# angeladai/sgnn

Measured on AMD Instinct MI355X. Metric: TSDF blocks/sec fwd+bwd (64^3@5% occ, bs32), higher is better.
Workload: dtype f32

## Files before the change

### sgnn_amd/csrc/conv.hip

```cpp
#include <stdlib.h>
#include "common.h"

#include "conv_common.h"

#define CONV_SMALL_GRID ((int64_t)((g_tune.conv_small_rows + CONV_ROWS_PER_BLOCK - 1) / CONV_ROWS_PER_BLOCK))

template <int CIN, int COUT, int M, bool EX, bool WEPI>
__device__ __forceinline__ void conv_fwd_body(const float *__restrict__ x, int64_t n_in,
                                              const float *__restrict__ w, const int32_t *__restrict__ table,
                                              int64_t ld, int K, int64_t n_out, float *y, int flags,
                                              int in_shift, const ConvEx &ex, const ConvEpi &epi, int wg_cap) {
  using C = ConvCfg<CIN, COUT>;
  constexpr int V = C::V, CINP = C::CINP, NT = C::NT, KC = C::KC;
  constexpr int RPW = 16 * M;
  __shared__ __attribute__((aligned(16))) float wl[KC * C::PER_K];
  __shared__ double sred[4 * 2 * NT * 16];
  static_assert(!WEPI || (NT == 1 && M == 4 && !EX && COUT % 4 == 0), "wide epilogue: one column tile of whole 16-byte chunks");
  __shared__ float ecst[WEPI ? 64 : 1];

  const int tid = threadIdx.x, lane = tid & 63, wave = tid >> 6;
  const int r = lane & 15, q = lane >> 4;
  const unsigned groups = EX ? (unsigned)ex.groups : 1u;
  unsigned nwg = gridDim.x;
  if (epi.n_dev) n_out = sgnn_dyn_n(n_out, epi.n_dev);
// ... 144 lines not shown
      load_b(0, b0);
      int kk = 0;
      for (; kk + 1 < kc; kk += 2) {
        gather(iv1, a1);
        const int32_t iv3 = idx_at(k0 + kk + 3);
        load_b(kk + 1, b1);
        __builtin_amdgcn_sched_barrier(0);
        mma_b(a0, b0);
        __builtin_amdgcn_sched_barrier(0);
        gather(iv2, a0);
        iv1 = iv3;
        iv2 = idx_at(k0 + kk + 4);
        load_b(kk + 2 < kc ? kk + 2 : kc - 1, b0);
        __builtin_amdgcn_sched_barrier(0);
        mma_b(a1, b1);
        __builtin_amdgcn_sched_barrier(0);
      }
      if constexpr (WEPI) {
        __builtin_amdgcn_sched_barrier(0);
        if constexpr (SGNN_WEPI_EARLY != 0) conv_epi_wide_prefetch<COUT, M>(erows, row0, n_out, epi, epi.stats, x, SGNN_WEPI_EARLY);
        __builtin_amdgcn_sched_barrier(0);
      }
      if (kk < kc) mma_b(a0, b0);
    }
  }

  if constexpr (WEPI)
    conv_epi_wide_finish<COUT, M>(acc, erows, row0, n_out, y, epi, epi.stats, ecst, s1, s2, x);
  else
    conv_epilogue_rows<COUT, M, NT>(acc, row0, n_out, groups, grp, y, epi, EX ? 0 : epi.stats, x, s1, s2);
  }
  conv_epilogue_stats<COUT, NT>(s1, s2, epi, EX ? 0 : epi.stats, sred, blockIdx.x);
}

template <int CIN, int COUT, int M, bool EX>
__global__ __launch_bounds__(256) void k_conv_fwd(const float *__restrict__ x, int64_t n_in,
                                                 const float *__restrict__ w, const int32_t *__restrict__ table,
                                                 int64_t ld, int K, int64_t n_out, float *y, int flags,
                                                 int in_shift, ConvEx ex, ConvEpi epi, int wg_cap) {
  conv_fwd_body<CIN, COUT, M, EX, false>(x, n_in, w, table, ld, K, n_out, y, flags, in_shift, ex, epi, wg_cap);
}

template <int CIN, int COUT>
__global__ __launch_bounds__(256) __attribute__((amdgpu_waves_per_eu(4, 8))) void k_conv_fwd_w(
    const float *__restrict__ x, int64_t n_in, const float *__restrict__ w, const int32_t *__restrict__ table, int64_t ld,
    int K, int64_t n_out, float *y, int flags, int in_shift, ConvEx ex, ConvEpi epi, int wg_cap) {
  conv_fwd_body<CIN, COUT, CONV_MREP, false, true>(x, n_in, w, table, ld, K, n_out, y, flags, in_shift, ex, epi, wg_cap);
}

template <int CIN, int COUT>
__global__ __launch_bounds__(256) void k_conv_small(const float *__restrict__ x, int64_t n_in,
                                                   const float *__restrict__ w, const int32_t *__restrict__ table,
                                                   int64_t ld, int K, int64_t n_out, float *y, int flags, int in_shift,
                                                   ConvEpi epi) {
  using C = ConvCfg<CIN, COUT>;
  constexpr int V = C::V, CINP = C::CINP, NT = C::NT;
  constexpr int KW = 7;
  __shared__ float red[4][NT * 256];
  __shared__ double sred[4][2][NT * 16];
  const int tid = threadIdx.x, lane = tid & 63, wave = tid >> 6;
  const int r = lane & 15, q = lane >> 4;
  const int64_t row0 = (int64_t)blockIdx.x * 16;
  if (epi.n_dev) {
    n_out = sgnn_dyn_n(n_out, epi.n_dev);
    if (row0 >= n_out) {
      if (epi.stats)
        for (int o = tid; o < 2 * COUT; o += 256) epi.partial[(size_t)blockIdx.x * 2 * COUT + o] = 0.0;
      return;
    }
  }
  const bool transpose = flags & SGNN_CONV_TRANSPOSE_W, flip = flags & SGNN_CONV_FLIP_K;
  const int per = (K + 3) >> 2;
  const int k0 = wave * per;
  const int nk = (K - k0) < per ? ((K - k0) > 0 ? (K - k0) : 0) : per;

  const uint32_t ldx4 = (uint32_t)epi.ldx * 4u, ldy4 = (uint32_t)epi.ldy * 4u;
  const __amdgpu_buffer_rsrc_t rs_x = make_rsrc(x, (uint32_t)(((n_in - 1) * epi.ldx + CIN) * 4));
  const __amdgpu_buffer_rsrc_t rs_t = make_rsrc(table, (uint32_t)((int64_t)K * ld * 4));
  const __amdgpu_buffer_rsrc_t rs_y = make_rsrc(y, (uint32_t)(((n_out - 1) * epi.ldy + COUT) * 4));
  const uint32_t lane_off = (uint32_t)(row0 + r) * 4u;
  const uint32_t ld4 = (uint32_t)ld * 4u;

  int32_t id[KW];
#pragma unroll
  for (int kk = 0; kk < KW; ++kk) {
    const int k = k0 + (kk < nk ? kk : (nk > 0 ? nk - 1 : 0));
    id[kk] = (int32_t)__builtin_amdgcn_raw_buffer_load_b32(rs_t, lane_off, (k < K ? k : K - 1) * ld4, 0) >> in_shift;
  }
  float a[KW][V];
#pragma unroll
  for (int kk = 0; kk < KW; ++kk) buf_load_floats<V>(rs_x, (uint32_t)id[kk] * ldx4 + (uint32_t)(q * V * 4), a[kk]);
  float b[KW][NT][V];
  if (transpose) {
    const __amdgpu_buffer_rsrc_t rs_w = make_rsrc(w, (uint32_t)((int64_t)K * CIN * COUT * 4));
#pragma unroll
    for (int kk = 0; kk < KW; ++kk) {
      const int k = k0 + kk;
      const int ks = flip ? (K - 1 - k) : k;
#pragma unroll
      for (int nt = 0; nt < NT; ++nt) {
        const int n = nt * 16 + r;
        const bool okw = kk < nk && n < COUT;
        buf_load_floats<V>(rs_w, okw ? (uint32_t)((ks * COUT + n) * CIN + q * V) * 4u : 0xFFFFF800u, b[kk][nt]);
        if constexpr (CINP != CIN) {
#pragma unroll
          for (int s = 0; s < V; ++s)
            if (3 * V + s >= CIN) b[kk][nt][s] = (q >= conv_first_pad_quarter<CIN, V>(s)) ? 0.f : b[kk][nt][s];
        }
      }
    }
  } else if constexpr (V == 4 && CIN <= 16 && (CIN * COUT) % 4 == 0) {
    constexpr int SL = CIN * COUT, G4 = SL / 4, NL = (G4 + 63) / 64;
    static_assert(SL <= NT * 256, "the weight slice must fit the wave's partial-tile buffer");
    float *ws = red[wave];
    const __amdgpu_buffer_rsrc_t rs_w = make_rsrc(w, (uint32_t)((int64_t)K * SL * 4));
    float g[KW][NL][4];
#pragma unroll
    for (int kk = 0; kk < KW; ++kk) {
      const int k = k0 + kk;
      const int ks = flip ? (K - 1 - k) : k;
#pragma unroll
      for (int l = 0; l < NL; ++l) {
        const int e4 = l * 64 + lane;
        buf_load_floats<4>(rs_w, (kk < nk && e4 < G4) ? (uint32_t)(ks * SL + e4 * 4) * 4u : 0xFFFFF800u, g[kk][l]);
      }
    }
    auto wave_sync = [] {
      __builtin_amdgcn_fence(__ATOMIC_RELEASE, "wavefront");
      __builtin_amdgcn_wave_barrier();
      __builtin_amdgcn_fence(__ATOMIC_ACQUIRE, "wavefront");
    };
#pragma unroll
    for (int kk = 0; kk < KW; ++kk) {
      wave_sync();
#pragma unroll
      for (int l = 0; l < NL; ++l) {
        const int e4 = l * 64 + lane;
        if (e4 < G4) {
#pragma unroll
          for (int j = 0; j < 4; ++j) ws[e4 * 4 + j] = g[kk][l][j];
        }
      }
      wave_sync();
#pragma unroll
      for (int nt = 0; nt < NT; ++nt) {
        const int n = nt * 16 + r;
#pragma unroll
        for (int s = 0; s < V; ++s) {
          const int c = q * V + s;
          b[kk][nt][s] = (c < CIN && n < COUT) ? ws[c * COUT + n] : 0.f;
        }
      }
    }
  } else {
#pragma unroll
    for (int kk = 0; kk < KW; ++kk) {
      const int k = k0 + kk;
      const int ks = flip ? (K - 1 - k) : k;
#pragma unroll
      for (int nt = 0; nt < NT; ++nt) {
        const int n = nt * 16 + r;
#pragma unroll
        for (int s = 0; s < V; ++s) {
          const int c = q * V + s;
          float v = 0.f;
          if (kk < nk && c < CIN && n < COUT) v = w[((int64_t)ks * CIN + c) * COUT + n];
          b[kk][nt][s] = v;
        }
      }
    }
  }
  if constexpr (CINP != CIN) {
#pragma unroll
    for (int kk = 0; kk < KW; ++kk)
#pragma unroll
      for (int s = 0; s < V; ++s)
        if (3 * V + s >= CIN) a[kk][s] = (q >= conv_first_pad_quarter<CIN, V>(s)) ? 0.f : a[kk][s];
  }
  f32x4 acc[2][NT];
#pragma unroll
  for (int h = 0; h < 2; ++h)
#pragma unroll
    for (int nt = 0; nt < NT; ++nt) acc[h][nt] = f32x4{0.f, 0.f, 0.f, 0.f};
#pragma unroll
  for (int kk = 0; kk < KW; ++kk) {
    if (kk < nk) {
#pragma unroll
      for (int s = 0; s < V; ++s)
#pragma unroll
        for (int nt = 0; nt < NT; ++nt)
          acc[kk & 1][nt] = __builtin_amdgcn_mfma_f32_16x16x4f32(a[kk][s], b[kk][nt][s], acc[kk & 1][nt], 0, 0, 0);
    }
  }
#pragma unroll
  for (int nt = 0; nt < NT; ++nt)
#pragma unroll
    for (int i = 0; i < 4; ++i) red[wave][nt * 256 + (q * 4 + i) * 16 + r] = acc[0][nt][i] + acc[1][nt][i];
  __syncthreads();

  const bool has_add = epi.addend != nullptr;
  const __amdgpu_buffer_rsrc_t rs_a =
      make_rsrc(has_add ? epi.addend : x, has_add ? (uint32_t)(((n_out - 1) * epi.ld_add + COUT) * 4) : 0u);
  const uint32_t lda4 = (uint32_t)epi.ld_add * 4u;
  const int stats = epi.stats;
  const __amdgpu_buffer_rsrc_t rs_b =
      make_rsrc(stats == 2 ? epi.bn_x : x, stats == 2 ? (uint32_t)(((n_out - 1) * epi.ld_bnx + COUT) * 4) : 0u);
  const uint32_t ldb4 = (uint32_t)epi.ld_bnx * 4u;
  const int orow_l = tid >> 4, ocol_l = tid & 15;
  const int64_t row = row0 + orow_l;
#pragma unroll
  for (int nt = 0; nt < NT; ++nt) {
    const int col = nt * 16 + ocol_l;
    const bool ok = col < COUT && row < n_out;
    const int e = nt * 256 + orow_l * 16 + ocol_l;
    float v = (red[0][e] + red[1][e]) + (red[2][e] + red[3][e]);
    const uint32_t orow = (uint32_t)row;
    if (has_add) v += __uint_as_float(__builtin_amdgcn_raw_buffer_load_b32(rs_a, ok ? orow * lda4 + col * 4u : 0xFFFFFFFFu, 0, 0));
    __builtin_amdgcn_raw_buffer_store_b32(__float_as_uint(v), rs_y, ok ? orow * ldy4 + col * 4u : 0xFFFFFFFFu, 0, 0);
    if (stats) {
      double f1 = 0.0, f2 = 0.0;
      if (stats == 1) {
        f1 = ok ? (double)v : 0.0;
        f2 = f1 * f1;
      } else {
        float cm = 0.f, ci = 0.f, cg = 1.f, cb = 0.f;
        if (col < COUT) {
          cm = epi.mean[col];
          ci = epi.invstd[col];
          cg = epi.gamma ? epi.gamma[col] : 1.f;
          cb = epi.beta ? epi.beta[col] : 0.f;
        }
        const float xb = __uint_as_float(__builtin_amdgcn_raw_buffer_load_b32(rs_b, ok ? orow * ldb4 + col * 4u : 0xFFFFFFFFu, 0, 0));
        const float xh = (xb - cm) * ci;
        const float t = fmaf(xh, cg, cb);
        const float dz = ok ? (t > 0.f ? v : v * epi.leak) : 0.f;
        f1 = (double)dz;
        f2 = (double)dz * (double)xh;
      }
      f1 += __shfl_xor(f1, 16); f2 += __shfl_xor(f2, 16);
      f1 += __shfl_xor(f1, 32); f2 += __shfl_xor(f2, 32);
      if (lane < 16) {
        sred[wave][0][nt * 16 + lane] = f1;
        sred[wave][1][nt * 16 + lane] = f2;
      }
    }
  }
  if (stats) {
    __syncthreads();
    for (int o = tid; o < 2 * NT * 16; o += 256) {
      const int which = o / (NT * 16), col = o % (NT * 16);
      if (col < COUT)
        epi.partial[((size_t)blockIdx.x * 2 + which) * COUT + col] =
            (sred[0][which][col] + sred[1][which][col]) + (sred[2][which][col] + sred[3][which][col]);
    }
  }
}

__global__ __launch_bounds__(256) void k_conv_fwd_generic(const float *__restrict__ x, int cin,
                                                         const float *__restrict__ w, int K,
                                                         const int32_t *__restrict__ table, int64_t ld,
                                                         int64_t n_out, int cout, float *__restrict__ y,
                                                         int flags, int in_shift, ConvEx ex, const int64_t *n_dev) {
  n_out = sgnn_dyn_n(n_out, n_dev);
  const int64_t t = (int64_t)blockIdx.x * 256 + threadIdx.x;
  if (t >= n_out * ex.groups * cout) return;
  const int64_t orow = t / cout;
  const int n = (int)(t - orow * cout);
  const int64_t row = orow / ex.groups;
  const int grp = (int)(orow - row * ex.groups);
  w += (int64_t)grp * K * cin * cout;
  const bool transpose = flags & SGNN_CONV_TRANSPOSE_W, flip = flags & SGNN_CONV_FLIP_K;
  float acc = 0.f;
  for (int k = 0; k < K; ++k) {
    const int32_t idx = table[(int64_t)(ex.kmap ? ex.kmap[grp * K + k] : k) * ld + row];
    if (idx < 0) continue;
    const float *xr = x + ((int64_t)(idx >> in_shift) * ex.in_mul + (ex.kadd ? ex.kadd[grp * K + k] : 0)) * cin;
    const int ks = flip ? (K - 1 - k) : k;
    for (int c = 0; c < cin; ++c) {
      const float wv = transpose ? w[((int64_t)ks * cout + n) * cin + c] : w[((int64_t)ks * cin + c) * cout + n];
      acc = fmaf(xr[c], wv, acc);
    }
  }
  y[t] = acc;
}

#define CONV_EX_CASES(X) \
  X(48, 16) X(16, 48) X(24, 8) X(8, 24) X(16, 24) X(24, 16) X(24, 32) X(32, 24) X(64, 32) X(32, 64) X(56, 28) X(28, 56)

#define CONV_FWD_CASES(X) \
  X(1, 8) X(8, 8) X(8, 12) X(12, 12) X(12, 16) X(16, 16) X(34, 16) X(30, 16) X(26, 16) X(48, 16) \
  X(8, 1) X(12, 8) X(16, 12) X(16, 34) X(16, 30) X(16, 26) X(16, 48) X(32, 16) X(16, 32) X(4, 16) X(16, 4) \
  X(16, 24) X(24, 16) X(24, 32) X(32, 24) X(64, 32) X(32, 64) X(56, 28) X(28, 56) X(32, 32) X(28, 16) X(16, 28)

int64_t sgnn_conv_grid_blocks(int64_t n_out, int cin, int cout, int K) {
  const int64_t grid4 = (n_out + CONV_ROWS_PER_BLOCK - 1) / CONV_ROWS_PER_BLOCK;
  if (grid4 < CONV_SMALL_GRID) return (n_out + 15) / 16;
  return grid4;
}


bool sgnn_conv_u_supported(int cin, int cout, int K);
bool sgnn_conv_u_launch(const float *x, int64_t n_in, int cin, const float *w, int K, const int32_t *table, int64_t ld,
                        int64_t n_out, int cout, float *y, int flags, int in_shift, const ConvEpi &epi, hipStream_t s);

bool conv_wide_epi_ok(const ConvEpi &epi, const float *y, int K) {
  if (!g_tune.conv_wide_epi || K > 27 || (epi.ldy & 3) || ((uintptr_t)y & 15)) return false;
  if (epi.addend && ((epi.ld_add & 3) || ((uintptr_t)epi.addend & 15))) return false;
  if (epi.stats == 2 && ((epi.ld_bnx & 3) || ((uintptr_t)epi.bn_x & 15))) return false;
  return true;
}
template <int CI, int CO, bool EXV>
static void conv_launch_big(unsigned grid4, hipStream_t s, const float *x, int64_t n_in, const float *w, const int32_t *table,
                            int64_t ld, int K, int64_t n_out, float *y, int flags, int in_shift, const ConvEx &ex,
                            const ConvEpi &epi) {
  if constexpr (!EXV && CO % 4 == 0 && CO <= 16 && CI <= 16) {
    static_assert(ConvCfg<CI, CO>::KC >= 27, "one weight chunk holds a 3x3x3 filter");
    if (conv_wide_epi_ok(epi, y, K)) {
      SGNN_LAUNCH((k_conv_fwd_w<CI, CO>), dim3(grid4), dim3(256), 0, s, x, n_in, w, table, ld, K, n_out, y, flags, in_shift,
                  ex, epi, !g_tune.conv_one_round ? 0 : conv_wg_capacity<k_conv_fwd_w<CI, CO>>());
      return;
    }
  }
  SGNN_LAUNCH((k_conv_fwd<CI, CO, CONV_MREP, EXV>), dim3(grid4), dim3(256), 0, s, x, n_in, w, table, ld, K, n_out, y,
              flags, in_shift, ex, epi,
              (EXV || !g_tune.conv_one_round) ? 0 : conv_wg_capacity<k_conv_fwd<CI, CO, CONV_MREP, EXV>>());
}

bool sgnn_conv_epi_supported(int cin, int cout) {
#define X(CI, CO) \
  if (cin == CI && cout == CO) return true;
  CONV_FWD_CASES(X)
#undef X
  return false;
}

int sgnn_conv_fwd_impl(const float *x, int64_t n_in, int cin, const float *w, int K, const int32_t *table, int64_t ld,
                       int64_t n_out, int cout, float *y, int flags, int in_shift, const int32_t *kmap,
                       const int32_t *kadd, int in_mul, int groups, int table_rows, const ConvEpi *epi_in,
                       sgnn_stream_t stream) {
  SGNN_CHECK_ARG(cin >= 1 && cout >= 1 && K >= 1 && K <= 64 && n_out >= 0 && ld >= n_out && in_shift >= 0 &&
                 in_shift < 31 && in_mul >= 1 && groups >= 1 && groups <= 64 && table_rows >= 1 &&
                 table_rows <= 64 && (kmap || table_rows >= K));
  if (n_out == 0) return SGNN_OK;
  SGNN_CHECK_ARG(x && w && table && y && n_in >= 1);
  SGNN_CHECK_ARG(ld % CONV_ROWS_PER_BLOCK == 0);
  ConvEpi epi{};
  if (epi_in) epi = *epi_in;
  if (epi.ldx <= 0) epi.ldx = cin;
  if (epi.ldy <= 0) epi.ldy = cout;
  if (epi.ld_add <= 0) epi.ld_add = cout;
  if (epi.ld_bnx <= 0) epi.ld_bnx = cout;
  const bool plain = !kmap && !kadd && in_mul == 1 && groups == 1 && table_rows == K;
  const bool has_epi = epi.ldx != cin || epi.ldy != cout || epi.addend || epi.stats;
  SGNN_CHECK_ARG(epi.ldx >= cin && epi.ldx <= 1024 && epi.ldy >= cout && epi.ldy <= 1024 && epi.ld_add >= cout &&
                 epi.ld_add <= 1024 && epi.ld_bnx >= cout && epi.ld_bnx <= 1024);
  SGNN_CHECK_ARG(epi.stats >= 0 && epi.stats <= 2 && (!epi.stats || (plain && epi.partial)));
  SGNN_CHECK_ARG(epi.stats != 2 || (epi.bn_x && epi.mean && epi.invstd));
  SGNN_CHECK_ARG(!epi.stats || K <= 28);
  const int64_t lmax = epi.ldy > epi.ld_add ? (epi.ldy > epi.ld_bnx ? epi.ldy : epi.ld_bnx)
                                            : (epi.ld_add > epi.ld_bnx ? epi.ld_add : epi.ld_bnx);
  if (n_in * epi.ldx * 4 > 0xFFFFF000ll || n_out * groups * lmax * 4 > 0xFFFFF000ll ||
      (int64_t)table_rows * ld * 4 > 0xFFFFF000ll) {
    sgnn_set_error("sgnn_conv_fwd: a slab exceeds the 4 GiB raw-buffer window (n_in=%lld cin=%d n_out=%lld cout=%d)",
                   (long long)n_in, cin, (long long)n_out, cout);
    return SGNN_EOVERFLOW;
  }
  hipStream_t s = (hipStream_t)stream;
  const ConvEx ex{kmap, kadd, in_mul, groups, table_rows};
  const unsigned grid4 = (unsigned)((n_out + CONV_ROWS_PER_BLOCK - 1) / CONV_ROWS_PER_BLOCK) * (unsigned)groups;
  const unsigned grid1 = (unsigned)((n_out + 63) / 64) * (unsigned)groups;
  const bool small = grid4 < CONV_SMALL_GRID;
  bool done = false;
  const int prof = sgnn_prof_begin_launch(0, n_out * groups, cin, cout, K, flags, s);
#define LAUNCH_FWD(CI, CO, EXV)                                                                         \
  do {                                                                                                  \
    if (small && !EXV && K <= 28 && (g_tune.conv_small || epi.stats))                                      \
      SGNN_LAUNCH((k_conv_small<CI, CO>), dim3((unsigned)((n_out + 15) / 16)), dim3(256), 0, s,         \
                         x, n_in, w, table, ld, K, n_out, y, flags, in_shift, epi);                     \
    else if (small)                                                                                     \
      SGNN_LAUNCH((k_conv_fwd<CI, CO, 1, EXV>), dim3(grid1), dim3(256), 0, s, x, n_in, w, table,        \
                         ld, K, n_out, y, flags, in_shift, ex, epi, 0);                                 \
    else                                                                                                \
      conv_launch_big<CI, CO, EXV>(grid4, s, x, n_in, w, table, ld, K, n_out, y, flags, in_shift, ex, epi); \
    done = true;                                                                                        \
  } while (0)
  if (plain && !small && g_tune.conv_unrolled && sgnn_conv_u_supported(cin, cout, K))
    done = sgnn_conv_u_launch(x, n_in, cin, w, K, table, ld, n_out, cout, y, flags, in_shift, epi, s);
#define X(CI, CO) \
  if (!done && plain && cin == CI && cout == CO) LAUNCH_FWD(CI, CO, false);
  CONV_FWD_CASES(X)
#undef X
#define X(CI, CO) \
  if (!done && !plain && cin == CI && cout == CO) LAUNCH_FWD(CI, CO, true);
  CONV_EX_CASES(X)
#undef X
  if (!done) {
    if (has_epi) {
      sgnn_set_error("sgnn_conv_fwd_epi: strided / fused epilogues need one of the compiled (cin, cout) shapes, got (%d, %d)", cin, cout);
      return SGNN_EINVAL;
    }
    const int64_t total = n_out * groups * cout;
    SGNN_LAUNCH(k_conv_fwd_generic, dim3((unsigned)((total + 255) / 256)), dim3(256), 0, s, x, cin, w, K,
                       table, ld, n_out, cout, y, flags, in_shift, ex, epi.n_dev);
  }
  sgnn_prof_end_launch(prof, s);
  SGNN_CHECK_LAUNCH();
  return SGNN_OK;
}

SGNN_EXPORT int sgnn_conv_fwd_ex(const float *x, int64_t n_in, int cin, const float *w, int K, const int32_t *table,
                                 int64_t ld, int64_t n_out, int cout, float *y, int flags, int in_shift,
                                 const int32_t *kmap, const int32_t *kadd, int in_mul, int groups,
                                 int table_rows, sgnn_stream_t stream) {
  return sgnn_conv_fwd_impl(x, n_in, cin, w, K, table, ld, n_out, cout, y, flags, in_shift, kmap, kadd, in_mul,
                            groups, table_rows, nullptr, stream);
}

SGNN_EXPORT int sgnn_conv_fwd(const float *x, int64_t n_in, int cin, const float *w, int K, const int32_t *table,
                              int64_t ld, int64_t n_out, int cout, float *y, int flags, int in_shift,
                              sgnn_stream_t stream) {
  return sgnn_conv_fwd_impl(x, n_in, cin, w, K, table, ld, n_out, cout, y, flags, in_shift, nullptr, nullptr, 1, 1,
                            K, nullptr, stream);
}

SGNN_EXPORT int64_t sgnn_conv_stats_blocks(int64_t n_out) { return n_out > 0 ? sgnn_conv_grid_blocks(n_out, 0, 0, 0) : 0; }

SGNN_EXPORT int sgnn_conv_fwd_epi(const float *x, int64_t n_in, int cin, int64_t ldx, const float *w, int K,
                                  const int32_t *table, int64_t ld, int64_t n_out, int cout, float *y, int64_t ldy,
                                  int flags, const float *addend, int64_t ld_add, int stats, double *partial,
                                  const float *bn_x, int64_t ld_bnx, const float *mean, const float *invstd,
                                  const float *gamma, const float *beta, float leak, sgnn_stream_t stream) {
  ConvEpi epi{ldx, ldy, ld_add, addend, stats, partial, bn_x, ld_bnx, mean, invstd, gamma, beta, leak, nullptr};
  return sgnn_conv_fwd_impl(x, n_in, cin, w, K, table, ld, n_out, cout, y, flags, 0, nullptr, nullptr, 1, 1, K, &epi,
                            stream);
}

__device__ int32_t g_expand_maps[192];

int sgnn_expand_maps(const int32_t **S, const int32_t **ST, const int32_t **PAR) {
  static const int32_t *base = nullptr;
  if (!base) {
    int32_t host[192];
    for (int g = 0; g < 8; ++g)
      for (int i = 0; i < 8; ++i) {
        const int o0 = ((i >> 2) & 1) - 1 + ((g >> 2) & 1), o1 = ((i >> 1) & 1) - 1 + ((g >> 1) & 1),
                  o2 = (i & 1) - 1 + (g & 1);
        const int srow = (o0 + 1) * 9 + (o1 + 1) * 3 + (o2 + 1);
        host[g * 8 + i] = srow;
        host[64 + g * 8 + i] = 26 - srow;
        host[128 + g * 8 + i] = g;
      }
    SGNN_HIP_TRY(hipMemcpyToSymbol(HIP_SYMBOL(g_expand_maps), host, sizeof(host)));
    void *p = nullptr;
    SGNN_HIP_TRY(hipGetSymbolAddress(&p, HIP_SYMBOL(g_expand_maps)));
    base = (const int32_t *)p;
  }
  *S = base;
  *ST = base + 64;
  *PAR = base + 128;
  return SGNN_OK;
}

__device__ __forceinline__ void axis_taps(int j, int i, int &lo, int &hi) {
  if (j == 0) { lo = i ? 0 : -1; hi = i ? 1 : -1; }
  else        { lo = i ? 1 : -1; hi = i ? 1 : 0; }
}

__global__ __launch_bounds__(256) void k_expand_weights(const float *__restrict__ w, int cc, float *__restrict__ wc) {
  const int t = blockIdx.x * 256 + threadIdx.x;
  if (t >= 64 * cc) return;
  const int gi = t / cc, e = t - gi * cc, g = gi >> 3, i = gi & 7;
  int l0, h0, l1, h1, l2, h2;
  axis_taps((g >> 2) & 1, (i >> 2) & 1, l0, h0);
  axis_taps((g >> 1) & 1, (i >> 1) & 1, l1, h1);
  axis_taps(g & 1, i & 1, l2, h2);
  float acc = 0.f;
  for (int dz = l0; dz <= h0; ++dz)
    for (int dy = l1; dy <= h1; ++dy)
      for (int dx = l2; dx <= h2; ++dx) acc += w[(size_t)((dz + 1) * 9 + (dy + 1) * 3 + (dx + 1)) * cc + e];
  wc[t] = acc;
}

__global__ __launch_bounds__(256) void k_expand_weights_bwd(const float *__restrict__ dwc, int cc,
                                                           float *__restrict__ dw) {
  const int t = blockIdx.x * 256 + threadIdx.x;
  if (t >= 27 * cc) return;
  const int tap = t / cc, e = t - tap * cc;
  const int d0 = tap / 9 - 1, d1 = (tap / 3) % 3 - 1, d2 = tap % 3 - 1;
  float acc = 0.f;
  for (int g = 0; g < 8; ++g) {
    const int j0 = (g >> 2) & 1, j1 = (g >> 1) & 1, j2 = g & 1;
    const int i0 = j0 ? (d0 > 0) : (d0 >= 0), i1 = j1 ? (d1 > 0) : (d1 >= 0), i2 = j2 ? (d2 > 0) : (d2 >= 0);
    acc += dwc[(size_t)(g * 8 + i0 * 4 + i1 * 2 + i2) * cc + e];
  }
  dw[t] = acc;
}

SGNN_EXPORT int sgnn_expand_weights(const float *w, int cin, int cout, float *wc, sgnn_stream_t stream) {
  SGNN_CHECK_ARG(w && wc && cin >= 1 && cout >= 1);
  const int cc = cin * cout;
  SGNN_LAUNCH(k_expand_weights, dim3((64 * cc + 255) / 256), dim3(256), 0, (hipStream_t)stream, w, cc, wc);
  SGNN_CHECK_LAUNCH();
  return SGNN_OK;
}

SGNN_EXPORT int sgnn_expand_weights_bwd(const float *dwc, int cin, int cout, float *dw, sgnn_stream_t stream) {
  SGNN_CHECK_ARG(dwc && dw && cin >= 1 && cout >= 1);
  const int cc = cin * cout;
  SGNN_LAUNCH(k_expand_weights_bwd, dim3((27 * cc + 255) / 256), dim3(256), 0, (hipStream_t)stream, dwc, cc, dw);
  SGNN_CHECK_LAUNCH();
  return SGNN_OK;
}

template <int CIN, int COUT>
struct DwCfg {
  static constexpr int MT = (CIN + 15) / 16, NT = (COUT + 15) / 16;
  static constexpr int KPB = (MT * NT == 1) ? 9 : ((MT * NT <= 3) ? 5 : 3);
};

#ifndef DW_PAIR
#define DW_PAIR 1
#endif
template <int CIN, int COUT, bool EX, int KPBT = 0>
__global__ __launch_bounds__(256) void k_conv_dw(const float *__restrict__ x, int64_t n_in,
                                                const float *__restrict__ dy, const int32_t *__restrict__ table,
                                                int64_t ld, int K, int64_t n_out, float *__restrict__ partial,
                                                int64_t rows_per_block, int in_shift, ConvEx ex, int64_t ldx,
                                                int64_t ld_dy, const int64_t *n_dev) {
  if (n_dev) {
    n_out = sgnn_dyn_n(n_out, n_dev);
    const int64_t per = (n_out + gridDim.x - 1) / gridDim.x;
    rows_per_block = ((per + 255) / 256) * 256;
    if (rows_per_block < 256) rows_per_block = 256;
  }
  constexpr int MT = (CIN + 15) / 16, NT = (COUT + 15) / 16;
  constexpr int DW_KPB = KPBT > 0 ? KPBT : DwCfg<CIN, COUT>::KPB;
  constexpr int V = (CIN + 3) / 4, CINP = 4 * V;
  constexpr int W = (COUT + 3) / 4, COUTP = 4 * W;
  constexpr int XS = 64 * CINP, YS = 64 * COUTP;
  constexpr bool PAIR = DW_PAIR && MT * NT == 1 && CIN == 8 && KPBT == 0 && !EX;
  constexpr int XT = PAIR ? 2 : 1;
  constexpr int RED = DW_KPB * MT * 16 * NT * 16;
  constexpr int LDS_FLOATS = (4 * (XT * XS + YS) > RED) ? 4 * (XT * XS + YS) : RED;
  __shared__ __attribute__((aligned(16))) float lds[LDS_FLOATS];

  const int tid = threadIdx.x, lane = tid & 63, wave = tid >> 6;
  const int i16 = lane & 15, q = lane >> 4;
  const unsigned lin = sgnn_xcd_tile(blockIdx.y * gridDim.x + blockIdx.x, gridDim.x * gridDim.y);
  const unsigned bx = lin / gridDim.y, by = lin % gridDim.y;
  const unsigned groups = EX ? (unsigned)ex.groups : 1u;
  const unsigned kgroups = gridDim.y / groups;
  const unsigned grp = by / kgroups;
  const int k0 = (by % kgroups) * DW_KPB;
  const int32_t *kmap = (EX && ex.kmap) ? ex.kmap + grp * K : nullptr;
  const int table_rows = EX ? ex.table_rows : K;
  const int kc = (K - k0) < DW_KPB ? (K - k0) : DW_KPB;
  const int64_t blk_row0 = (int64_t)bx * rows_per_block;
  int64_t blk_row1 = blk_row0 + rows_per_block;
  if (blk_row1 > n_out) blk_row1 = n_out;

  const uint32_t ldx4 = (uint32_t)ldx * 4u;
  const __amdgpu_buffer_rsrc_t rs_x = make_rsrc(x, (uint32_t)(((n_in - 1) * ldx + CIN) * 4));
  const __amdgpu_buffer_rsrc_t rs_t = make_rsrc(table, (uint32_t)((int64_t)table_rows * ld * 4));
  const __amdgpu_buffer_rsrc_t rs_dy = make_rsrc(dy, (uint32_t)(((n_out * groups - 1) * ld_dy + COUT) * 4));
  const uint32_t ld4 = (uint32_t)ld * 4u;
  float *xs = lds + wave * (XT * XS + YS);
  float *ys = xs + XT * XS;

  constexpr int NP = (DW_KPB + 1) / 2;
  f32x4 accp[PAIR ? NP : 1];
#pragma unroll
  for (int p = 0; p < (PAIR ? NP : 1); ++p) accp[p] = f32x4{0.f, 0.f, 0.f, 0.f};
  f32x4 acc[DW_KPB][MT][NT];
#pragma unroll
  for (int kk = 0; kk < DW_KPB; ++kk)
#pragma unroll
    for (int mt = 0; mt < MT; ++mt)
#pragma unroll
      for (int nt = 0; nt < NT; ++nt) acc[kk][mt][nt] = f32x4{0.f, 0.f, 0.f, 0.f};

  constexpr bool RCX = (CIN == 16 || CIN == 8);
  constexpr int LPR = RCX ? CIN / 4 : 1, RPI = 64 / LPR, NI = RCX ? LPR : 4, GW = RCX ? 4 : V;
  const int rc_row = lane / LPR, rc_chunk = lane % LPR;
  auto gather = [&](int32_t iv, float(&g)[NI][GW]) {
#pragma unroll
    for (int m = 0; m < NI; ++m) {
      const int32_t id = __builtin_amdgcn_ds_bpermute((RCX ? m * RPI + rc_row : m * 16 + i16) * 4, iv);
      buf_load_floats<GW>(rs_x, (uint32_t)id * ldx4 + (uint32_t)(RCX ? rc_chunk * 16 : q * V * 4), g[m]);
    }
  };
  auto norm_rows = [&](float(&g)[NI][GW]) {
    if constexpr (CINP != CIN) {
#pragma unroll
      for (int m = 0; m < NI; ++m)
#pragma unroll
        for (int s = 0; s < GW; ++s)
          if (3 * V + s >= CIN) g[m][s] = (q == 3) ? 0.f : g[m][s];
    }
  };
  auto store_rows = [&](const float(&g)[NI][GW]) {
#pragma unroll
    for (int m = 0; m < NI; ++m) {
      float *p = RCX ? xs + (m * RPI + rc_row) * CINP + rc_chunk * 4 : xs + (m * 16 + i16) * CINP + q * V;
#pragma unroll
      for (int s = 0; s < GW; ++s) p[s] = g[m][s];
    }
  };
  auto store_rows_to = [&](const float(&g)[NI][GW], float *tile) {
#pragma unroll
    for (int m = 0; m < NI; ++m) {
      float *p = tile + (m * RPI + rc_row) * CINP + rc_chunk * 4;
#pragma unroll
      for (int s = 0; s < GW; ++s) p[s] = g[m][s];
    }
  };
  auto mma_pair = [&](int p, const float(&b)[16][NT]) {
    const float *src = xs + (i16 >> 3) * XS + (i16 & 7);
#pragma unroll
    for (int t = 0; t < 16; ++t) {
      const float a = ((i16 & 7) < CINP) ? src[(4 * t + q) * CINP] : 0.f;
      accp[p] = __builtin_amdgcn_mfma_f32_16x16x4f32(a, b[t][0], accp[p], 0, 0, 0);
    }
  };
  auto mma_chunk = [&](int kk, const float(&b)[16][NT]) {
#pragma unroll
    for (int t = 0; t < 16; ++t) {
      float a[MT];
#pragma unroll
      for (int mt = 0; mt < MT; ++mt) {
        const int ch = mt * 16 + i16;
        a[mt] = (ch < CINP) ? xs[(4 * t + q) * CINP + ch] : 0.f;
      }
#pragma unroll
      for (int mt = 0; mt < MT; ++mt)
#pragma unroll
        for (int nt = 0; nt < NT; ++nt)
          acc[kk][mt][nt] = __builtin_amdgcn_mfma_f32_16x16x4f32(a[mt], b[t][nt], acc[kk][mt][nt], 0, 0, 0);
    }
  };

  for (int64_t base = blk_row0 + wave * 64; base < blk_row1; base += 256) {
    int32_t idxv[DW_KPB];
#pragma unroll
    for (int kk = 0; kk < DW_KPB; ++kk) {
      const int ko = k0 + (kk < kc ? kk : kc - 1);
      int32_t id;
      if constexpr (EX) {
        const int trow = kmap ? kmap[ko] : ko;
        id = (int32_t)__builtin_amdgcn_raw_buffer_load_b32(rs_t, (uint32_t)(base + lane) * 4u, trow * ld4, 0);
        id = (id >> in_shift) * ex.in_mul + ((ex.kadd && id >= 0) ? ex.kadd[grp * K + ko] : 0);
      } else {
        id = (int32_t)__builtin_amdgcn_raw_buffer_load_b32(rs_t, (uint32_t)(base + lane) * 4u, ko * ld4, 0) >> in_shift;
      }
      idxv[kk] = (kk < kc) ? id : -1;
    }
    if constexpr (COUT == 16 || COUT == 8) {
      constexpr int LY = COUT / 4, RY = 64 / LY;
      const int yr = lane / LY, yc = lane % LY;
      float g[LY][4];
#pragma unroll
      for (int m = 0; m < LY; ++m) {
        const int64_t row = base + m * RY + yr;
        const uint32_t off = (row < blk_row1) ? (uint32_t)((row * groups + grp) * ld_dy + yc * 4) * 4u : 0xFFFFF800u;
        buf_load_floats<4>(rs_dy, off, g[m]);
      }
#pragma unroll
      for (int m = 0; m < LY; ++m) {
        float *p = ys + (m * RY + yr) * COUTP + yc * 4;
#pragma unroll
        for (int s = 0; s < 4; ++s) p[s] = g[m][s];
      }
    } else {
      float g[4][W];
#pragma unroll
      for (int m = 0; m < 4; ++m) {
        const int64_t row = base + m * 16 + i16;
        const uint32_t off =
            (row < blk_row1) ? (uint32_t)((row * groups + grp) * ld_dy + q * W) * 4u : 0xFFFFF800u;
        buf_load_floats<W>(rs_dy, off, g[m]);
        if constexpr (COUTP != COUT) {
#pragma unroll
          for (int s = 0; s < W; ++s)
            if (3 * W + s >= COUT) g[m][s] = (q == 3) ? 0.f : g[m][s];
        }
      }
#pragma unroll
      for (int m = 0; m < 4; ++m) {
        float *p = ys + (m * 16 + i16) * COUTP + q * W;
#pragma unroll
        for (int s = 0; s < W; ++s) p[s] = g[m][s];
// ... 390 lines not shown
```

### sgnn_amd/csrc/conv_unrolled.hip

```cpp
#include "conv_common.h"

template <int CIN, int COUT, int K, bool WEPI>
__device__ __forceinline__ void conv_fwd_u_body(const float *__restrict__ x, int64_t n_in, const float *__restrict__ w,
                                                const int32_t *__restrict__ table, int64_t ld, int64_t n_out, float *y,
                                                int flags, int in_shift, const ConvEpi &epi, int wg_cap) {
  using C = ConvCfg<CIN, COUT>;
  constexpr int V = C::V, CINP = C::CINP, NT = C::NT, M = 4;
  constexpr int KC = C::KC27 < K ? C::KC27 : K;
  static_assert(KC < 27 || C::RESIDENT_BYTES <= 80 * 1024 || (CIN == 16 && COUT == 34), "resident weight image costs a workgroup per CU");
  __shared__ __attribute__((aligned(16))) float wl[KC * C::PER_K];
  __shared__ double sred[4 * 2 * NT * 16];
  static_assert(!WEPI || (NT == 1 && COUT % 4 == 0), "wide epilogue: one column tile of whole 16-byte chunks");
  __shared__ float ecst[WEPI ? 64 : 1];

  const int tid = threadIdx.x, lane = tid & 63, wave = tid >> 6;
  const int r = lane & 15, q = lane >> 4;
  unsigned nwg = gridDim.x;
  if (epi.n_dev) n_out = sgnn_dyn_n(n_out, epi.n_dev);
  int J = 1;
  if (wg_cap > 0) {
    J = (int)(((n_out + 255) / 256 + wg_cap - 1) / wg_cap);
    if (J < 1) J = 1;
  }
  if (epi.n_dev || J > 1) {
    nwg = (unsigned)((n_out + 256 * (int64_t)J - 1) / (256 * (int64_t)J));
    if (blockIdx.x >= nwg) {
      if (epi.stats)
        for (int o = tid; o < 2 * COUT; o += 256) epi.partial[(size_t)blockIdx.x * 2 * COUT + o] = 0.0;
      return;
    }
  }
  const unsigned tile = sgnn_xcd_tile(blockIdx.x, nwg);
  const bool transpose = flags & SGNN_CONV_TRANSPOSE_W, flip = flags & SGNN_CONV_FLIP_K;

  const uint32_t ldx4 = (uint32_t)epi.ldx * 4u;
  const __amdgpu_buffer_rsrc_t rs_x = make_rsrc(x, (uint32_t)(((n_in - 1) * epi.ldx + CIN) * 4));
  const __amdgpu_buffer_rsrc_t rs_t = make_rsrc(table, (uint32_t)((int64_t)K * ld * 4));
  const uint32_t ld4 = (uint32_t)ld * 4u;
  int perm[M];
#pragma unroll
  for (int m = 0; m < M; ++m) perm[m] = (m * 16 + r) * 4;
  double s1[NT], s2[NT];
#pragma unroll
  for (int nt = 0; nt < NT; ++nt) s1[nt] = s2[nt] = 0.0;
  int32_t idx[K];
  f32x4 acc[M][NT];
  if constexpr (WEPI) conv_epi_wide_constants<COUT>(ecst, epi, epi.stats);

  float a[2][M][V];
  auto gather = [&](int k) {
#pragma unroll
    for (int m = 0; m < M; ++m) {
      const int32_t id = __builtin_amdgcn_ds_bpermute(perm[m], idx[k]);
      buf_load_floats<V>(rs_x, (uint32_t)id * ldx4 + (uint32_t)(q * V * 4), a[k & 1][m]);
    }
  };
  auto stage = [&](int k0) {
    conv_stage_weights<CIN, COUT>(wl, w, K, k0, (K - k0) < KC ? (K - k0) : KC, transpose, flip);
  };
  float bf[2][NT][V];
  auto load_b = [&](int k) {
    const int kk = k % KC;
#pragma unroll
    for (int nt = 0; nt < NT; ++nt) {
      const float *bp = wl + (kk * NT * 16 + nt * 16 + r) * CINP + q * V;
#pragma unroll
      for (int s = 0; s < V; ++s) bf[k & 1][nt][s] = bp[s];
    }
  };
  auto mma = [&](int k) {
    const float(&b)[NT][V] = bf[k & 1];
#pragma unroll
    for (int s = 0; s < V; ++s)
#pragma unroll
      for (int m = 0; m < M; ++m) {
        float av = a[k & 1][m][s];
        if constexpr (CINP != CIN)
          if (3 * V + s >= CIN) av = (q >= conv_first_pad_quarter<CIN, V>(s)) ? 0.f : av;
#pragma unroll
        for (int nt = 0; nt < NT; ++nt)
          acc[m][nt] = __builtin_amdgcn_mfma_f32_16x16x4f32(av, b[nt][s], acc[m][nt], 0, 0, 0);
      }
  };

  for (int j = 0; j < J; ++j) {
  const int64_t wg_row0 = ((int64_t)tile * J + j) * 256;
  if (j > 0 && wg_row0 >= n_out) break;
  const int64_t row0 = wg_row0 + wave * 64;
  const uint32_t lane_off = (uint32_t)(row0 + lane) * 4u;
#pragma unroll
  for (int k = 0; k < K; ++k)
    idx[k] = (int32_t)__builtin_amdgcn_raw_buffer_load_b32(rs_t, lane_off, k * ld4, 0) >> in_shift;
#pragma unroll
  for (int m = 0; m < M; ++m)
#pragma unroll
    for (int nt = 0; nt < NT; ++nt) acc[m][nt] = f32x4{0.f, 0.f, 0.f, 0.f};
  gather(0);
  EpiRows<WEPI ? M : 1> erows;
#pragma unroll
  for (int k = 0; k < K; ++k) {
    if (k % KC == 0) {
      if (KC < K || j == 0) stage(k);
      load_b(k);
    }
    if (k + 1 < K) gather(k + 1);
    if (k + 1 < K && (k + 1) % KC != 0) load_b(k + 1);
    if constexpr (WEPI) {
      if (k == K - 1) conv_epi_wide_prefetch<COUT, M>(erows, row0, n_out, epi, epi.stats, x);
    }
    __builtin_amdgcn_sched_barrier(0);
    mma(k);
    __builtin_amdgcn_sched_barrier(0);
  }

  if constexpr (WEPI)
    conv_epi_wide_finish<COUT, M>(acc, erows, row0, n_out, y, epi, epi.stats, ecst, s1, s2, x);
  else
    conv_epilogue_rows<COUT, M, NT>(acc, row0, n_out, 1u, 0u, y, epi, epi.stats, x, s1, s2);
  }
  conv_epilogue_stats<COUT, NT>(s1, s2, epi, epi.stats, sred, blockIdx.x);
}

template <int CIN, int COUT, int K>
__global__ __launch_bounds__(256) void k_conv_fwd_u(const float *__restrict__ x, int64_t n_in, const float *__restrict__ w,
                                                   const int32_t *__restrict__ table, int64_t ld, int64_t n_out, float *y,
                                                   int flags, int in_shift, ConvEpi epi, int wg_cap) {
  conv_fwd_u_body<CIN, COUT, K, false>(x, n_in, w, table, ld, n_out, y, flags, in_shift, epi, wg_cap);
}

template <int CIN, int COUT>
__global__ __launch_bounds__(256) __attribute__((amdgpu_waves_per_eu(4, 8))) void k_conv_fwd_uw(
    const float *__restrict__ x, int64_t n_in, const float *__restrict__ w, const int32_t *__restrict__ table, int64_t ld,
    int64_t n_out, float *y, int flags, int in_shift, ConvEpi epi, int wg_cap) {
  conv_fwd_u_body<CIN, COUT, 8, true>(x, n_in, w, table, ld, n_out, y, flags, in_shift, epi, wg_cap);
}

#define CONV_U_CASES_27(X) X(34, 16) X(16, 34) X(30, 16) X(16, 30) X(26, 16) X(16, 26)
#define CONV_U_CASES_8(X) X(8, 8) X(8, 12) X(12, 8) X(12, 12) X(12, 16) X(16, 12) X(16, 16)

bool sgnn_conv_u_supported(int cin, int cout, int K) {
#define X(CI, CO) \
  if (K == 27 && cin == CI && cout == CO) return true;
  CONV_U_CASES_27(X)
#undef X
#define X(CI, CO) \
  if (K == 8 && cin == CI && cout == CO) return true;
  CONV_U_CASES_8(X)
#undef X
  return false;
}

bool conv_wide_epi_ok(const ConvEpi &epi, const float *y, int K);

template <int CI, int CO, int KK>
static void conv_u_launch_plain(unsigned grid, hipStream_t s, const float *x, int64_t n_in, const float *w, const int32_t *table,
                                int64_t ld, int64_t n_out, float *y, int flags, int in_shift, const ConvEpi &epi) {
  if constexpr (KK == 8 && CO % 4 == 0 && CO <= 16) {
    if (conv_wide_epi_ok(epi, y, KK)) {
      SGNN_LAUNCH((k_conv_fwd_uw<CI, CO>), dim3(grid), dim3(256), 0, s, x, n_in, w, table, ld, n_out, y, flags, in_shift, epi,
                  g_tune.conv_one_round ? conv_wg_capacity<k_conv_fwd_uw<CI, CO>>() : 0);
      return;
    }
  }
  SGNN_LAUNCH((k_conv_fwd_u<CI, CO, KK>), dim3(grid), dim3(256), 0, s, x, n_in, w, table, ld, n_out, y, flags, in_shift,
              epi, g_tune.conv_one_round ? conv_wg_capacity<k_conv_fwd_u<CI, CO, KK>>() : 0);
}

bool sgnn_conv_u_launch(const float *x, int64_t n_in, int cin, const float *w, int K, const int32_t *table, int64_t ld,
                        int64_t n_out, int cout, float *y, int flags, int in_shift, const ConvEpi &epi, hipStream_t s) {
  const unsigned grid = (unsigned)((n_out + 255) / 256);
#define X(CI, CO)                                                                                    \
  if (K == 27 && cin == CI && cout == CO) {                                                          \
    conv_u_launch_plain<CI, CO, 27>(grid, s, x, n_in, w, table, ld, n_out, y, flags, in_shift, epi); \
    return true;                                                                                     \
  }
  CONV_U_CASES_27(X)
#undef X
#define X(CI, CO)                                                                                   \
  if (K == 8 && cin == CI && cout == CO) {                                                          \
    conv_u_launch_plain<CI, CO, 8>(grid, s, x, n_in, w, table, ld, n_out, y, flags, in_shift, epi); \
    return true;                                                                                    \
  }
  CONV_U_CASES_8(X)
#undef X
  return false;
}
```

Measured before the change: 5716.

## Add unrolled software-pipelined kernel for grouped strided/transposed convolutions

Adds a specialised unrolled MFMA conv kernel for the strided/grouped (ex) paths with shapes 48->16 K8 and 16->48 K16. It keeps the whole per-group weight image resident in LDS, gathers input rows D steps ahead and double-buffers the B operand so that gathers overlap the MFMAs. The aim is to cut the latency stalls of the generic ex kernel. In exchange it uses more registers and LDS, and it only covers two specific configurations.

```diff
diff --git a/sgnn_amd/csrc/conv.hip b/sgnn_amd/csrc/conv.hip
--- a/sgnn_amd/csrc/conv.hip
+++ b/sgnn_amd/csrc/conv.hip
@@ -470,6 +470,9 @@
 bool sgnn_conv_u_supported(int cin, int cout, int K);
 bool sgnn_conv_u_launch(const float *x, int64_t n_in, int cin, const float *w, int K, const int32_t *table, int64_t ld,
                         int64_t n_out, int cout, float *y, int flags, int in_shift, const ConvEpi &epi, hipStream_t s);
+bool sgnn_conv_ux_launch(const float *x, int64_t n_in, int cin, const float *w, int K, const int32_t *table, int64_t ld,
+                         int64_t n_out, int cout, float *y, int flags, int in_shift, const ConvEx &ex, const ConvEpi &epi,
+                         hipStream_t s);
 
 bool conv_wide_epi_ok(const ConvEpi &epi, const float *y, int K) {
   if (!g_tune.conv_wide_epi || K > 27 || (epi.ldy & 3) || ((uintptr_t)y & 15)) return false;
@@ -554,6 +557,8 @@
   } while (0)
   if (plain && !small && g_tune.conv_unrolled && sgnn_conv_u_supported(cin, cout, K))
     done = sgnn_conv_u_launch(x, n_in, cin, w, K, table, ld, n_out, cout, y, flags, in_shift, epi, s);
+  if (!plain && !small && g_tune.conv_unrolled)
+    done = sgnn_conv_ux_launch(x, n_in, cin, w, K, table, ld, n_out, cout, y, flags, in_shift, ex, epi, s);
 #define X(CI, CO) \
   if (!done && plain && cin == CI && cout == CO) LAUNCH_FWD(CI, CO, false);
   CONV_FWD_CASES(X)
diff --git a/sgnn_amd/csrc/conv_unrolled.hip b/sgnn_amd/csrc/conv_unrolled.hip
--- a/sgnn_amd/csrc/conv_unrolled.hip
+++ b/sgnn_amd/csrc/conv_unrolled.hip
@@ -150,6 +150,114 @@
   return false;
 }
 
+template <int CIN, int COUT, int K, int D, bool KADD>
+__global__ __launch_bounds__(256) __attribute__((amdgpu_waves_per_eu(3, 8))) void k_conv_fwd_ux(const float *__restrict__ x, int64_t n_in, const float *__restrict__ w,
+                                                    const int32_t *__restrict__ table, int64_t ld, int64_t n_out, float *y,
+                                                    int flags, int in_shift, ConvEx ex, ConvEpi epi) {
+  using C = ConvCfg<CIN, COUT>;
+  constexpr int V = C::V, CINP = C::CINP, NT = C::NT, M = 4;
+  static_assert(CINP == CIN && NT * 16 == COUT, "unpadded shapes only (no zero pass, no pad-channel select)");
+  static_assert(K * C::PER_K * 4 <= (160 * 1024) / 3, "resident weight image costs a workgroup per CU");
+  static_assert(D >= 1 && D < K, "prefetch distance");
+  __shared__ __attribute__((aligned(16))) float wl[K * C::PER_K];
+
+  const int tid = threadIdx.x, lane = tid & 63, wave = tid >> 6;
+  const int r = lane & 15, q = lane >> 4;
+  const unsigned groups = (unsigned)ex.groups;
+  unsigned nwg = gridDim.x;
+  if (epi.n_dev) {
+    n_out = sgnn_dyn_n(n_out, epi.n_dev);
+    nwg = (unsigned)((n_out + 255) / 256) * groups;
+    if (blockIdx.x >= nwg) return;
+  }
+  const unsigned lin = sgnn_xcd_tile(blockIdx.x, nwg);
+  const unsigned tile = lin / groups, grp = lin % groups;
+  const int64_t row0 = ((int64_t)tile * 4 + wave) * 64;
+  w += (int64_t)grp * K * CIN * COUT;
+  const int32_t *kmap = ex.kmap + grp * K;
+  const int32_t *kadd = KADD ? ex.kadd + grp * K : nullptr;
+  const bool transpose = flags & SGNN_CONV_TRANSPOSE_W, flip = flags & SGNN_CONV_FLIP_K;
+
+  const uint32_t ldx4 = (uint32_t)epi.ldx * 4u;
+  const __amdgpu_buffer_rsrc_t rs_x = make_rsrc(x, (uint32_t)(((n_in - 1) * epi.ldx + CIN) * 4));
+  const __amdgpu_buffer_rsrc_t rs_t = make_rsrc(table, (uint32_t)((int64_t)ex.table_rows * ld * 4));
+  const uint32_t lane_off = (uint32_t)(row0 + lane) * 4u, ld4 = (uint32_t)ld * 4u;
+  int perm[M];
+#pragma unroll
+  for (int m = 0; m < M; ++m) perm[m] = (m * 16 + r) * 4;
+
+  int32_t idx[K];
+#pragma unroll
+  for (int k = 0; k < K; ++k) {
+    const int32_t id = (int32_t)__builtin_amdgcn_raw_buffer_load_b32(rs_t, lane_off, kmap[k] * ld4, 0);
+    idx[k] = (id >> in_shift) * ex.in_mul + ((KADD && id >= 0) ? kadd[k] : 0);
+  }
+  f32x4 acc[M][NT];
+#pragma unroll
+  for (int m = 0; m < M; ++m)
+#pragma unroll
+    for (int nt = 0; nt < NT; ++nt) acc[m][nt] = f32x4{0.f, 0.f, 0.f, 0.f};
+
+  float a[D + 1][M][V];
+  auto gather = [&](int k) {
+#pragma unroll
+    for (int m = 0; m < M; ++m) {
+      const int32_t id = __builtin_amdgcn_ds_bpermute(perm[m], idx[k]);
+      buf_load_floats<V>(rs_x, (uint32_t)id * ldx4 + (uint32_t)(q * V * 4), a[k % (D + 1)][m]);
+    }
+  };
+  float bf[2][NT][V];
+  auto load_b = [&](int k) {
+#pragma unroll
+    for (int nt = 0; nt < NT; ++nt) {
+      const float *bp = wl + (k * NT * 16 + nt * 16 + r) * CINP + q * V;
+#pragma unroll
+      for (int s = 0; s < V; ++s) bf[k & 1][nt][s] = bp[s];
+    }
+  };
+  auto mma = [&](int k) {
+#pragma unroll
+    for (int s = 0; s < V; ++s)
+#pragma unroll
+      for (int m = 0; m < M; ++m)
+#pragma unroll
+        for (int nt = 0; nt < NT; ++nt)
+          acc[m][nt] = __builtin_amdgcn_mfma_f32_16x16x4f32(a[k % (D + 1)][m][s], bf[k & 1][nt][s], acc[m][nt], 0, 0, 0);
+  };
+
+#pragma unroll
+  for (int k = 0; k < D; ++k) gather(k);
+  conv_stage_weights<CIN, COUT>(wl, w, K, 0, K, transpose, flip);
+  load_b(0);
+#pragma unroll
+  for (int k = 0; k < K; ++k) {
+    if (k + D < K) gather(k + D);
+    if (k + 1 < K) load_b(k + 1);
+    __builtin_amdgcn_sched_barrier(0);
+    mma(k);
+    __builtin_amdgcn_sched_barrier(0);
+  }
+  double s1[NT], s2[NT];
+  conv_epilogue_rows<COUT, M, NT>(acc, row0, n_out, groups, grp, y, epi, 0, x, s1, s2);
+}
+
+bool sgnn_conv_ux_launch(const float *x, int64_t n_in, int cin, const float *w, int K, const int32_t *table, int64_t ld,
+                         int64_t n_out, int cout, float *y, int flags, int in_shift, const ConvEx &ex, const ConvEpi &epi,
+                         hipStream_t s) {
+  const unsigned grid = (unsigned)((n_out + 255) / 256) * (unsigned)ex.groups;
+  if (cin == 48 && cout == 16 && K == 8 && ex.groups == 8 && ex.kmap && !ex.kadd && ex.in_mul == 1) {
+    SGNN_LAUNCH((k_conv_fwd_ux<48, 16, 8, 1, false>), dim3(grid), dim3(256), 0, s, x, n_in, w, table, ld, n_out, y, flags,
+                in_shift, ex, epi);
+    return true;
+  }
+  if (cin == 16 && cout == 48 && K == 16 && ex.groups == 4 && ex.kmap && ex.kadd && ex.in_mul == 8) {
+    SGNN_LAUNCH((k_conv_fwd_ux<16, 48, 16, 2, true>), dim3(grid), dim3(256), 0, s, x, n_in, w, table, ld, n_out, y, flags,
+                in_shift, ex, epi);
+    return true;
+  }
+  return false;
+}
+
 bool conv_wide_epi_ok(const ConvEpi &epi, const float *y, int K);
 
 template <int CI, int CO, int KK>
```

New measurement: 5738, median of 5. Within noise of the previous version (+0.4%).
